# ParsaEsmati/SEA

Measured on AMD Instinct MI355X. Metric: rollout steps/sec (full-context forward, recompute mode) on cylinder_flow-shaped fields, higher is better.
Workload: dtype bf16

## Files before the change

sea_amd/csrc/mlp_block.hip:

```cpp
#include "gemm_core.hpp"
#include <stdlib.h>

struct MlpBlockLaunch {
    SeaMlpGroup g1[SEA_MAX_MLP_GROUPS];
    SeaMlp2Group g2[SEA_MAX_MLP_GROUPS];
    int tile_start[SEA_MAX_MLP_GROUPS + 1];
    int xcd_start[SEA_MAX_MLP_GROUPS + 1];
    int n_groups;
    float eps;
    int per_xcd;
    int probe;
};

__device__ __forceinline__ void glds16_blk(const void* gsrc, unsigned lds_addr) {
    unsigned keep;
    asm volatile("s_mov_b32 %0, m0\n\ts_mov_b32 m0, %2\n\ts_nop 0\n\tglobal_load_lds_dwordx4 %1, off\n\ts_mov_b32 m0, %0"
                 : "=&s"(keep) : "v"(gsrc), "s"(lds_addr) : "memory");
}

__device__ __forceinline__ void glds16_blk_s(const void* ubase, unsigned lane_off, unsigned lds_addr) {
    unsigned keep;
    asm volatile("s_mov_b32 %0, m0\n\ts_mov_b32 m0, %3\n\ts_nop 0\n\tglobal_load_lds_dwordx4 %1, %2\n\ts_mov_b32 m0, %0"
                 : "=&s"(keep) : "v"(lane_off), "s"(ubase), "s"(lds_addr) : "memory");
}

template <int KT, int NSB>
struct MlpBlockCfg {
    static constexpr int BM = 32, BKB = 128, NS = 4, NW = 8;
    static constexpr int E = KT * 64, S = NSB * 128;
    static constexpr int A_BYTES = KT * BM * BKB, STAGE = KT * 64 * BKB;
    static constexpr int PRM_OFF = A_BYTES + NS * STAGE;
    static constexpr int P1_BYTES = PRM_OFF + 2 * S * 4;
    static constexpr int SLAB_PITCH = 128 * 4 + 16, SLAB = BM * SLAB_PITCH;
    static constexpr int X3_OFF = NW * SLAB;
    static constexpr int RED2_OFF = X3_OFF + KT * BM * BKB;
    static constexpr int P2_BYTES = RED2_OFF + 2 * NW * BM * 4;
    static constexpr int RS = KT == 4 ? 8 : 4, SLOT = 16 * 128;
    static constexpr int RING_OFF = KT == 4 ? A_BYTES : P1_BYTES;
    static constexpr int RING_END = RING_OFF + NW * RS * SLOT;
    static constexpr int BYTES_ = P1_BYTES > P2_BYTES ? P1_BYTES : P2_BYTES;
    static constexpr int BYTES = BYTES_ > RING_END ? BYTES_ : RING_END;
};

__device__ __forceinline__ f32x4 mma16_first(const uint4& a, const uint4& b) {
    return __builtin_amdgcn_mfma_f32_16x16x32_bf16(__builtin_bit_cast(bf16x8, a), __builtin_bit_cast(bf16x8, b), f32x4{0.f, 0.f, 0.f, 0.f}, 0, 0, 0);
}

__device__ __forceinline__ constexpr int blk_col_base(int t, int half, int wq) { return (t >> 1) * 512 + half * 256 + wq * 64 + (t & 1) * 32; }

template <int KT, int NSB>
__global__ __launch_bounds__(512) void mlp_block_kernel(const MlpBlockLaunch L) {
    using T = __bf16;
    using Cf = MlpBlockCfg<KT, NSB>;
    constexpr int BM = 32, BKB = 128, BK = 64, NS = 4, NW = 8;
    constexpr int E = Cf::E, S = Cf::S, NSTAGE = S / 64, NT = NSB / 2;
    constexpr int A_BYTES = Cf::A_BYTES, STAGE = Cf::STAGE;
    constexpr int LPS = KT * 8 / NW;
    constexpr int PRM_OFF = Cf::PRM_OFF;
    constexpr int B1_OFF = 0, RED_OFF = S * 4;
    static_assert(RED_OFF + 2 * NW * BM * 4 <= A_BYTES && (S / 256) * 1024 <= A_BYTES && LPS * NW == KT * 8 && NT % 2 == 0 && Cf::BYTES <= 160 * 1024, "LDS layout of sea_mlp_block");
    static_assert((NT / 2) * 512 == S, "blk_col_base covers the hidden columns once");
    extern __shared__ __attribute__((aligned(16))) char smem[];
    int tile, gi = 0;
    if (L.per_xcd < 0) {
        const int xcd = (int)(blockIdx.x & 7), idx = (int)(blockIdx.x >> 3);
        if (xcd >= L.xcd_start[L.n_groups]) return;
        while (gi + 1 < L.n_groups && xcd >= L.xcd_start[gi + 1]) ++gi;
        tile = L.tile_start[gi] + (xcd - L.xcd_start[gi]) * 32 + idx;
        if (tile >= L.tile_start[gi + 1]) return;
    } else {
        tile = L.per_xcd > 0 ? (int)(blockIdx.x & 7) * L.per_xcd + (int)(blockIdx.x >> 3) : (int)blockIdx.x;
        if (tile >= L.tile_start[L.n_groups]) return;
        while (gi + 1 < L.n_groups && tile >= L.tile_start[gi + 1]) ++gi;
    }
    const SeaMlpGroup& G = L.g1[gi];
    const SeaMlp2Group& H = L.g2[gi];
    const int m0 = (tile - L.tile_start[gi]) * BM, M = G.M;
    const int tid = threadIdx.x, lane = tid & 63;
    const int wave = __builtin_amdgcn_readfirstlane(tid >> 6);
    const int r = lane & 15, g = lane >> 4;
    const int half = wave >> 2, wq = wave & 3;
    const T* A = static_cast<const T*>(G.A);
    const T* W = static_cast<const T*>(G.W1);
    const unsigned lds_base = __builtin_amdgcn_readfirstlane((unsigned)(uintptr_t)smem);
    const int rl = lane >> 3;
    const int chunk = (lane & 7) ^ (rl & 7);
    for (int p = wave; p < 2 * (S / 256); p += NW) {
        const float* src = p < S / 256 ? G.lnw : G.lnb;
        const int q = p < S / 256 ? p : p - S / 256;
        glds16_blk(src + q * 256 + lane * 4, lds_base + (unsigned)(PRM_OFF + p * 1024));
    }
    for (int p = wave; G.X32 == nullptr && p < KT * (BM / 8); p += NW) {
        const int kt = p / (BM / 8), u = p - kt * (BM / 8);
        int row = m0 + u * 8 + rl;
        row = row < M ? row : M - 1;
        glds16_blk(A + (int64_t)row * G.lda + kt * BK + chunk * 8, lds_base + (unsigned)(kt * BM * BKB + u * 8 * BKB));
    }
    const unsigned w1_lane = (unsigned)(((8 * (rl >> 2) + (rl & 3)) * G.ldw + chunk * 8) * 2);
    auto dma_stage = [&](int s) {
        const unsigned base = lds_base + (unsigned)(A_BYTES + (s % NS) * STAGE);
        const int t = s >> 2, u = (s >> 1) & 1, hs = s & 1;
#pragma unroll
        for (int i = 0; i < LPS; ++i) {
            const int p = i * NW + wave;
            const int kt = p >> 3, u8 = p & 7;
            const int urow = blk_col_base(t, hs, u8 >> 1) + 16 * (u8 & 1) + 4 * u;
            glds16_blk_s(W + (int64_t)urow * G.ldw + kt * BK, w1_lane, base + (unsigned)(kt * 64 * BKB + u8 * 8 * BKB));
        }
    };
    dma_stage(0);
    if (G.X32 != nullptr) {
        constexpr int CPT = E / 16;
        const int prow = tid >> 4, pl = tid & 15;
        int row = m0 + prow;
        row = row < M ? row : M - 1;
        const int c0 = pl * CPT;
        float xv[CPT];
#pragma unroll
        for (int c = 0; c < CPT; c += 4) load4(G.X32 + (int64_t)row * G.ldx32 + c0 + c, *reinterpret_cast<float(*)[4]>(xv + c));
        if (G.addend != nullptr) {
#pragma unroll
            for (int c = 0; c < CPT; c += 4) {
                float av[4];
                load4(G.addend + (int64_t)row * G.ldadd + c0 + c, av);
#pragma unroll
                for (int e = 0; e < 4; ++e) xv[c + e] += av[e];
            }
        }
        float gq[CPT], bq[CPT];
#pragma unroll
        for (int c = 0; c < CPT; c += 4) {
            load4(G.gamma + c0 + c, *reinterpret_cast<float(*)[4]>(gq + c));
#pragma unroll
            for (int e = 0; e < 4; ++e) bq[c + e] = 0.f;
            if (G.beta != nullptr) load4(G.beta + c0 + c, *reinterpret_cast<float(*)[4]>(bq + c));
            if (G.mod != nullptr) {
                float mw[4], mb[4];
                const T* mod = static_cast<const T*>(G.mod) + (int64_t)row * G.ldmod;
                load4(mod + c0 + c, mw);
                load4(mod + E + c0 + c, mb);
#pragma unroll
                for (int e = 0; e < 4; ++e) {
                    gq[c + e] += 1.0f + mw[e];
                    bq[c + e] += mb[e];
                }
            }
        }
        float s4[4] = {0.f, 0.f, 0.f, 0.f};
#pragma unroll
        for (int c = 0; c < CPT; c += 4)
#pragma unroll
            for (int e = 0; e < 4; ++e) s4[e] = add1(s4[e], xv[c + e]);
        float sm_ = add1(add1(s4[0], s4[1]), add1(s4[2], s4[3]));
#pragma unroll
        for (int o = 8; o >= 1; o >>= 1) sm_ += __shfl_xor(sm_, o);
        const float mean = sm_ * (1.0f / (float)E);
        float q4[4] = {0.f, 0.f, 0.f, 0.f};
#pragma unroll
        for (int c = 0; c < CPT; c += 4)
#pragma unroll
            for (int e = 0; e < 4; ++e) {
                const float d_ = xv[c + e] - mean;
                q4[e] = fma1(d_, d_, q4[e]);
            }
        float sq = add1(add1(q4[0], q4[1]), add1(q4[2], q4[3]));
#pragma unroll
        for (int o = 8; o >= 1; o >>= 1) sq += __shfl_xor(sq, o);
        const float rstd = 1.0f / sqrtf(sq * (1.0f / (float)E) + G.norm_eps);
#pragma unroll
        for (int c = 0; c < CPT; c += 8) {
            const int col = c0 + c, kt = col >> 6, ck = (col & 63) >> 3;
            bf16x8 pv;
#pragma unroll
            for (int e = 0; e < 8; ++e) pv[e] = (__bf16)((xv[c + e] - mean) * rstd * gq[c + e] + bq[c + e]);
            *reinterpret_cast<bf16x8*>(smem + kt * BM * BKB + prow * BKB + ((ck ^ (prow & 7)) << 4)) = pv;
        }
        asm volatile("s_waitcnt vmcnt(0) lgkmcnt(0)" ::: "memory");
    }
    for (int s = 1; s < NS - 1; ++s) dma_stage(s);

    const T* W2 = static_cast<const T*>(H.W2);
    const unsigned w2_lane = (unsigned)((rl * H.ldw2 + chunk * 8) * 2);
    const T* Wp = static_cast<const T*>(H.Wproj);
    const unsigned wp_lane = (unsigned)((rl * H.ldwp + chunk * 8) * 2);
    constexpr int NSLOT = (E / 16) * (NT / 2);
    constexpr int NJ = E / NW / 16;
    constexpr int NX = NJ * KT;
    auto w2_slot = [&](int k) {
        const unsigned dst = lds_base + (unsigned)(Cf::RING_OFF + (wave * Cf::RS + (k % Cf::RS)) * Cf::SLOT);
        if (k < NSLOT) {
            const int tau = k / (E / 16), j = k - tau * (E / 16);
            const T* ub = W2 + (int64_t)(j * 16) * H.ldw2 + blk_col_base(2 * tau, half, wq);
#pragma unroll
            for (int u = 0; u < 2; ++u)
                glds16_blk_s(ub + (int64_t)(8 * u) * H.ldw2, w2_lane, dst + (unsigned)(u * 1024));
        } else {
            const int kk = k - NSLOT, j = kk / KT, kt = kk - j * KT;
            const T* ub = Wp + (int64_t)(wave * (E / NW) + j * 16) * H.ldwp + kt * BK;
#pragma unroll
            for (int u = 0; u < 2; ++u)
                glds16_blk_s(ub + (int64_t)(8 * u) * H.ldwp, wp_lane, dst + (unsigned)(u * 1024));
        }
    };
    uint4 hid[NT][2];
    float mean[2], rstd[2];
    {
        f32x4 acc[NSB][2];
        uint4 areg[KT][2][2];
#pragma unroll
        for (int i = 0; i < NSB; ++i) {
            acc[i][0] = f32x4{0.f, 0.f, 0.f, 0.f};
            acc[i][1] = f32x4{0.f, 0.f, 0.f, 0.f};
        }
#pragma unroll
        for (int s = 0; s < NSTAGE; ++s) {
            if (s + 2 < NSTAGE) asm volatile("s_waitcnt vmcnt(%0) lgkmcnt(0)" ::"n"(2 * LPS) : "memory");
            else if (s + 1 < NSTAGE) asm volatile("s_waitcnt vmcnt(%0) lgkmcnt(0)" ::"n"(LPS) : "memory");
            else asm volatile("s_waitcnt vmcnt(0) lgkmcnt(0)" ::: "memory");
            __builtin_amdgcn_s_barrier();
            if (s + NS - 1 < NSTAGE) dma_stage(s + NS - 1);
            if (s == 0) {
                const char* sA = smem + r * BKB;
#pragma unroll
                for (int kt = 0; kt < KT; ++kt)
#pragma unroll
                    for (int kc = 0; kc < 2; ++kc) {
                        const int off = ((kc * 4 + g) ^ (r & 7)) << 4;
                        areg[kt][kc][0] = *reinterpret_cast<const uint4*>(sA + kt * BM * BKB + off);
                        areg[kt][kc][1] = *reinterpret_cast<const uint4*>(sA + kt * BM * BKB + 16 * BKB + off);
                    }
                asm volatile("s_waitcnt lgkmcnt(0)" ::: "memory");
            }
            if (s == 1)
                for (int p = wave; p < S / 256; p += NW) glds16_blk(G.b1 + p * 256 + lane * 4, lds_base + (unsigned)(B1_OFF + p * 1024));
            if ((s & 1) == half) {
                const char* sW = smem + A_BYTES + (s % NS) * STAGE + (wq * 16 + r) * BKB;
#pragma unroll
                for (int kt = 0; kt < KT; ++kt)
#pragma unroll
                    for (int kc = 0; kc < 2; ++kc) {
                        const int off = ((kc * 4 + g) ^ (r & 7)) << 4;
                        const uint4 wf = *reinterpret_cast<const uint4*>(sW + kt * 64 * BKB + off);
                        mma16<T>(wf, areg[kt][kc][0], acc[s >> 1][0]);
                        mma16<T>(wf, areg[kt][kc][1], acc[s >> 1][1]);
                    }
            }
        }
        if (L.probe == 1) return;
        float* red = reinterpret_cast<float*>(smem + RED_OFF);
        const float* pb1 = reinterpret_cast<const float*>(smem + B1_OFF);
        const float* pgm = reinterpret_cast<const float*>(smem + PRM_OFF);
        const float* pbt = pgm + S;
        const float inv_s = 1.0f / (float)S;
        float sum[2] = {0.f, 0.f};
#pragma unroll
        for (int i = 0; i < NSB; ++i) {
            const int n = blk_col_base(i >> 1, half, wq) + 8 * g + 4 * (i & 1);
            float bv[4];
            load4(pb1 + n, bv);
#pragma unroll
            for (int mb = 0; mb < 2; ++mb) {
#pragma unroll
                for (int q = 0; q < 4; ++q) acc[i][mb][q] += bv[q];
                sum[mb] += (acc[i][mb][0] + acc[i][mb][1]) + (acc[i][mb][2] + acc[i][mb][3]);
            }
        }
#pragma unroll
        for (int mb = 0; mb < 2; ++mb) {
            sum[mb] += __shfl_xor(sum[mb], 16);
            sum[mb] += __shfl_xor(sum[mb], 32);
            if (g == 0) red[wave * 32 + mb * 16 + r] = sum[mb];
        }
        __syncthreads();
#pragma unroll
        for (int k = 0; k < Cf::RS - 1; ++k) w2_slot(k);
        float sq[2] = {0.f, 0.f};
#pragma unroll
        for (int mb = 0; mb < 2; ++mb) {
            float t = 0.f;
#pragma unroll
            for (int w = 0; w < NW; ++w) t += red[w * 32 + mb * 16 + r];
            mean[mb] = t * inv_s;
        }
#pragma unroll
        for (int i = 0; i < NSB; ++i)
#pragma unroll
            for (int mb = 0; mb < 2; ++mb)
#pragma unroll
                for (int q = 0; q < 4; ++q) {
                    const float c = acc[i][mb][q] - mean[mb];
                    sq[mb] += c * c;
                }
#pragma unroll
        for (int mb = 0; mb < 2; ++mb) {
            sq[mb] += __shfl_xor(sq[mb], 16);
            sq[mb] += __shfl_xor(sq[mb], 32);
            if (g == 0) red[256 + wave * 32 + mb * 16 + r] = sq[mb];
        }
        asm volatile("s_waitcnt lgkmcnt(0)" ::: "memory");
        __builtin_amdgcn_s_barrier();
#pragma unroll
        for (int mb = 0; mb < 2; ++mb) {
            float t = 0.f;
#pragma unroll
            for (int w = 0; w < NW; ++w) t += red[256 + w * 32 + mb * 16 + r];
            rstd[mb] = 1.0f / sqrtf(t * inv_s + L.eps);
        }
#pragma unroll
        for (int i = 0; i < NSB; ++i) {
            const int n = blk_col_base(i >> 1, half, wq) + 8 * g + 4 * (i & 1);
            float gm[4], bt[4];
            load4(pgm + n, gm);
            load4(pbt + n, bt);
#pragma unroll
            for (int mb = 0; mb < 2; ++mb) {
                bf16x4 y;
#pragma unroll
                for (int q = 0; q < 4; ++q) y[q] = (__bf16)gelu_erf_bf16((acc[i][mb][q] - mean[mb]) * rstd[mb] * gm[q] + bt[q]);
                uint2 y2 = *reinterpret_cast<const uint2*>(&y);
                asm volatile("" : "+v"(y2.x), "+v"(y2.y));
                if (i & 1) {
                    hid[i >> 1][mb].z = y2.x;
                    hid[i >> 1][mb].w = y2.y;
                } else {
                    hid[i >> 1][mb].x = y2.x;
                    hid[i >> 1][mb].y = y2.y;
                }
            }
            __builtin_amdgcn_sched_barrier(0);
        }
    }
    __builtin_amdgcn_sched_barrier(0);
    if (L.probe == 2) {
        asm volatile("s_waitcnt vmcnt(0)" ::: "memory");
        return;
    }

    constexpr int NJB = E / 16;
    constexpr int NTOT = NSLOT + NX;
    f32x4 acc2[2][NJB];
    uint4 wp[KT * 2][NJ];
#pragma unroll
    for (int k = 0; k < NTOT; ++k) {
        const int tau = k / NJB, j = k - tau * NJB;
        {
            constexpr int AFTER_MAX = Cf::RS - 2;
            const int after = NTOT - 1 - k < AFTER_MAX ? NTOT - 1 - k : AFTER_MAX;
            switch (after) {
                case 6: asm volatile("s_waitcnt vmcnt(12) lgkmcnt(0)" ::: "memory"); break;
                case 5: asm volatile("s_waitcnt vmcnt(10) lgkmcnt(0)" ::: "memory"); break;
                case 4: asm volatile("s_waitcnt vmcnt(8) lgkmcnt(0)" ::: "memory"); break;
                case 3: asm volatile("s_waitcnt vmcnt(6) lgkmcnt(0)" ::: "memory"); break;
                case 2: asm volatile("s_waitcnt vmcnt(4) lgkmcnt(0)" ::: "memory"); break;
                case 1: asm volatile("s_waitcnt vmcnt(2) lgkmcnt(0)" ::: "memory"); break;
                default: asm volatile("s_waitcnt vmcnt(0) lgkmcnt(0)" ::: "memory"); break;
            }
        }
        if (k + Cf::RS - 1 < NTOT) w2_slot(k + Cf::RS - 1);
        const char* sl = smem + Cf::RING_OFF + (wave * Cf::RS + (k % Cf::RS)) * Cf::SLOT + r * 128;
        if (k >= NSLOT) {
            const int kk = k - NSLOT, jp = kk / KT, kt = kk - jp * KT;
#pragma unroll
            for (int kc = 0; kc < 2; ++kc) wp[kt * 2 + kc][jp] = *reinterpret_cast<const uint4*>(sl + (((kc * 4 + g) ^ (r & 7)) << 4));
            continue;
        }
#pragma unroll
        for (int u2 = 0; u2 < 2; ++u2) {
            const uint4 w = *reinterpret_cast<const uint4*>(sl + (((u2 * 4 + g) ^ (r & 7)) << 4));
            const int t = 2 * tau + u2;
            if (t == 0) {
                acc2[0][j] = mma16_first(w, hid[0][0]);
                acc2[1][j] = mma16_first(w, hid[0][1]);
            } else {
                mma16<T>(w, hid[t][0], acc2[0][j]);
                mma16<T>(w, hid[t][1], acc2[1][j]);
            }
        }
        __builtin_amdgcn_sched_barrier(0);
    }
    __syncthreads();
    if (L.probe == 3) return;
    {
    int tid_l = threadIdx.x;
    asm volatile("" : "+v"(tid_l));
    const int tid = tid_l, lane = tid & 63, r = lane & 15, g = lane >> 4;
    (void)lane;
    constexpr int NH = E / 128, JH = 8;
    const int srow = tid >> 4, scb = (tid & 15) * 8;
    float resv[NH][8];
    {
        int row = m0 + srow;
        row = row < M ? row : M - 1;
#pragma unroll
        for (int h = 0; h < NH; ++h) {
            const int col = h * 128 + scb;
            float b2a[4], b2b[4];
            load4(H.b2 + col, b2a);
            load4(H.b2 + col + 4, b2b);
            float ra[4], rb[4];
            if (H.R != nullptr) {
                load4(H.R + (int64_t)row * H.ldr + col, ra);
                load4(H.R + (int64_t)row * H.ldr + col + 4, rb);
            } else {
                load4(G.X32 + (int64_t)row * G.ldx32 + col, ra);
                load4(G.X32 + (int64_t)row * G.ldx32 + col + 4, rb);
                if (G.addend != nullptr) {
                    float aa[4], ab[4];
                    load4(G.addend + (int64_t)row * G.ldadd + col, aa);
                    load4(G.addend + (int64_t)row * G.ldadd + col + 4, ab);
#pragma unroll
                    for (int q = 0; q < 4; ++q) {
                        ra[q] += aa[q];
                        rb[q] += ab[q];
                    }
                }
            }
#pragma unroll
            for (int q = 0; q < 4; ++q) {
                resv[h][q] = b2a[q] + ra[q];
                resv[h][4 + q] = b2b[q] + rb[q];
            }
        }
    }
    constexpr int CPT = E / 16;
    const int ec0 = (tid & 15) * CPT;
    float ebp[CPT], egq[CPT], ebq[CPT];
    const bool has_norm = H.gamma != nullptr;
#pragma unroll
    for (int h = 0; h < NH; ++h) {
        char* slab = smem + wave * Cf::SLAB;
#pragma unroll
        for (int mb = 0; mb < 2; ++mb)
#pragma unroll
            for (int j = 0; j < JH; ++j)
                *reinterpret_cast<f32x4*>(slab + (mb * 16 + r) * Cf::SLAB_PITCH + (j * 16 + g * 4) * 4) = acc2[mb][h * JH + j];
        if (h == NH - 1) {
            __builtin_amdgcn_sched_barrier(0);
            int m = m0 + srow;
            m = m < M ? m : M - 1;
#pragma unroll
            for (int c = 0; c < CPT; c += 4) {
                load4(H.bproj + ec0 + c, *reinterpret_cast<float(*)[4]>(ebp + c));
#pragma unroll
                for (int q = 0; q < 4; ++q) egq[c + q] = ebq[c + q] = 0.f;
                if (has_norm) {
                    load4(H.gamma + ec0 + c, *reinterpret_cast<float(*)[4]>(egq + c));
                    if (H.beta != nullptr) load4(H.beta + ec0 + c, *reinterpret_cast<float(*)[4]>(ebq + c));
                    if (H.mod != nullptr) {
                        float mw[4], mb[4];
                        const T* mod = static_cast<const T*>(H.mod) + (int64_t)m * H.ldmod;
                        load4(mod + ec0 + c, mw);
                        load4(mod + E + ec0 + c, mb);
#pragma unroll
                        for (int q = 0; q < 4; ++q) {
                            egq[c + q] += 1.0f + mw[q];
                            ebq[c + q] += mb[q];
                        }
                    }
                }
            }
        }
        asm volatile("s_waitcnt lgkmcnt(0)" ::: "memory");
        __builtin_amdgcn_s_barrier();
        {
            float v[8];
#pragma unroll
            for (int q = 0; q < 8; ++q) v[q] = resv[h][q];
#pragma unroll
            for (int w = 0; w < NW; ++w) {
                const float4 a = *reinterpret_cast<const float4*>(smem + w * Cf::SLAB + srow * Cf::SLAB_PITCH + scb * 4);
                const float4 b = *reinterpret_cast<const float4*>(smem + w * Cf::SLAB + srow * Cf::SLAB_PITCH + scb * 4 + 16);
                v[0] += a.x; v[1] += a.y; v[2] += a.z; v[3] += a.w;
                v[4] += b.x; v[5] += b.y; v[6] += b.z; v[7] += b.w;
            }
            const int col = h * 128 + scb, kt = col >> 6, ck = (col & 63) >> 3;
            bf16x8 pv;
#pragma unroll
            for (int q = 0; q < 8; ++q) pv[q] = (__bf16)v[q];
            *reinterpret_cast<bf16x8*>(smem + Cf::X3_OFF + kt * BM * BKB + srow * BKB + ((ck ^ (srow & 7)) << 4)) = pv;
        }
        asm volatile("s_waitcnt lgkmcnt(0)" ::: "memory");
        __builtin_amdgcn_s_barrier();
        if (L.probe == 5 + h) return;
    }

    if (L.probe == 4) return;
    f32x4 acc3[2][NJ];
    {
        const char* sA = smem + Cf::X3_OFF + r * BKB;
#pragma unroll
        for (int kt = 0; kt < KT; ++kt)
#pragma unroll
            for (int kc = 0; kc < 2; ++kc) {
                const int off = ((kc * 4 + g) ^ (r & 7)) << 4;
                const uint4 af0 = *reinterpret_cast<const uint4*>(sA + kt * BM * BKB + off);
                const uint4 af1 = *reinterpret_cast<const uint4*>(sA + kt * BM * BKB + 16 * BKB + off);
#pragma unroll
                for (int j = 0; j < NJ; ++j) {
                    if (kt == 0 && kc == 0) {
                        acc3[0][j] = mma16_first(wp[0][j], af0);
                        acc3[1][j] = mma16_first(wp[0][j], af1);
                    } else {
                        mma16<T>(wp[kt * 2 + kc][j], af0, acc3[0][j]);
                        mma16<T>(wp[kt * 2 + kc][j], af1, acc3[1][j]);
                    }
                }
            }
    }
    constexpr int SEG = 80, YP = (E / 16) * SEG + 16;
    static_assert(BM * YP <= Cf::X3_OFF, "the y tile lies in front of the x3 tile");
#pragma unroll
    for (int i = 0; i < 2; ++i)
#pragma unroll
        for (int j = 0; j < NJ; ++j) {
            const int n = wave * (E / NW) + j * 16 + g * 4;
            *reinterpret_cast<f32x4*>(smem + (i * 16 + r) * YP + (n >> 4) * SEG + (n & 15) * 4) = acc3[i][j];
        }
    asm volatile("s_waitcnt lgkmcnt(0)" ::: "memory");
    __builtin_amdgcn_s_barrier();
    {
        float v[CPT];
#pragma unroll
        for (int c = 0; c < CPT; c += 4) {
            const float4 y = *reinterpret_cast<const float4*>(smem + srow * YP + ((ec0 + c) >> 4) * SEG + ((ec0 + c) & 15) * 4);
            v[c] = y.x + ebp[c]; v[c + 1] = y.y + ebp[c + 1]; v[c + 2] = y.z + ebp[c + 2]; v[c + 3] = y.w + ebp[c + 3];
        }
        if (has_norm) {
            float s4[4] = {0.f, 0.f, 0.f, 0.f};
#pragma unroll
            for (int c = 0; c < CPT; c += 4)
#pragma unroll
                for (int e = 0; e < 4; ++e) s4[e] = add1(s4[e], v[c + e]);
            float sm_ = add1(add1(s4[0], s4[1]), add1(s4[2], s4[3]));
#pragma unroll
            for (int o = 8; o >= 1; o >>= 1) sm_ += __shfl_xor(sm_, o);
            const float mean2 = sm_ * (1.0f / (float)E);
            float q4[4] = {0.f, 0.f, 0.f, 0.f};
#pragma unroll
            for (int c = 0; c < CPT; c += 4)
#pragma unroll
                for (int e = 0; e < 4; ++e) {
                    const float d_ = v[c + e] - mean2;
                    q4[e] = fma1(d_, d_, q4[e]);
                }
            float sq = add1(add1(q4[0], q4[1]), add1(q4[2], q4[3]));
#pragma unroll
            for (int o = 8; o >= 1; o >>= 1) sq += __shfl_xor(sq, o);
            const float rstd2 = 1.0f / sqrtf(sq * (1.0f / (float)E) + L.eps);
#pragma unroll
            for (int c = 0; c < CPT; ++c) v[c] = (v[c] - mean2) * rstd2 * egq[c] + ebq[c];
        }
        const int m = m0 + srow;
        if (m < M) {
#pragma unroll
            for (int c = 0; c < CPT; c += 4) {
                if (H.Y32 != nullptr) store4(H.Y32 + (int64_t)m * H.ldy32 + ec0 + c, v[c], v[c + 1], v[c + 2], v[c + 3]);
                if (H.Yact != nullptr) store4(static_cast<T*>(H.Yact) + (int64_t)m * H.ldyact + ec0 + c, v[c], v[c + 1], v[c + 2], v[c + 3]);
            }
        }
    }
    }
}

extern "C" int sea_mlp_block(const SeaMlpGroup* g1, const SeaMlp2Group* g2, int n_groups, float eps, int dtype, void* stream) {
    SEA_REQUIRE(g1 != nullptr && g2 != nullptr && n_groups >= 1 && n_groups <= SEA_MAX_MLP_GROUPS, "sea_mlp_block: n_groups=%d out of range", n_groups);
    const int E = g1[0].E, S = g1[0].S;
    const bool shape_ok = (E == 256 && S == 2048) || (E == 128 && S == 1024);
    if (dtype != SEA_BF16 || !shape_ok) {
        sea_set_error("sea_mlp_block: unsupported dtype / shape (dtype=%d E=%d S=%d): bf16, (E, S) in {(256, 2048), (128, 1024)}", dtype, E, S);
        return SEA_EUNSUPPORTED;
    }
    MlpBlockLaunch L;
    memset(&L, 0, sizeof(L));
    int total = 0;
    for (int i = 0; i < n_groups; ++i) {
        const SeaMlpGroup& G = g1[i];
        const SeaMlp2Group& H = g2[i];
        SEA_REQUIRE(G.E == E && G.S == S && H.E == E && H.S == S && G.M >= 1 && H.M == G.M, "sea_mlp_block[%d]: the groups of a launch share E and S; both halves the same M", i);
        SEA_REQUIRE((G.A || G.X32) && G.W1 && G.b1 && G.lnw && G.lnb, "sea_mlp_block[%d]: null pointer (first layer)", i);
        SEA_REQUIRE((G.X32 || (G.lda % 8 == 0 && G.lda >= E)) && G.ldw % 8 == 0 && G.ldw >= E, "sea_mlp_block[%d]: bad strides (first layer)", i);
        if (G.X32 != nullptr)
            SEA_REQUIRE(G.gamma && G.ldx32 % 4 == 0 && G.ldx32 >= E && (!G.addend || (G.ldadd % 4 == 0 && G.ldadd >= E)) && G.Xout == nullptr &&
                            (!G.mod || (G.ldmod % 8 == 0 && G.ldmod >= 2 * E)) && sea_aligned16(G.X32) && sea_aligned16(G.addend) && sea_aligned16(G.mod) &&
                            sea_aligned16(G.gamma) && sea_aligned16(G.beta) && G.norm_eps > 0.f,
                        "sea_mlp_block[%d]: norm prologue: null / misaligned pointer, bad stride, or Xout (the block keeps x + addend to itself)", i);
        SEA_REQUIRE(sea_aligned16(G.A) && sea_aligned16(G.W1) && sea_aligned16(G.b1) && sea_aligned16(G.lnw) && sea_aligned16(G.lnb), "sea_mlp_block[%d]: pointers must be 16-byte aligned", i);
        SEA_REQUIRE(H.W2 && H.b2 && (H.R || G.X32) && H.Wproj && H.bproj && (H.Y32 || H.Yact), "sea_mlp_block[%d]: null pointer (second layer; R may be NULL with the norm prologue: the residual is then x + addend)", i);
        SEA_REQUIRE(H.ldw2 % 8 == 0 && H.ldw2 >= S && H.ldwp % 8 == 0 && H.ldwp >= E && (!H.R || (H.ldr % 4 == 0 && H.ldr >= E)) &&
                        (!H.Y32 || (H.ldy32 % 4 == 0 && H.ldy32 >= E)) && (!H.Yact || (H.ldyact % 4 == 0 && H.ldyact >= E)) && (!H.mod || (H.ldmod % 4 == 0 && H.ldmod >= 2 * E)),
                    "sea_mlp_block[%d]: bad strides (second layer)", i);
        SEA_REQUIRE(sea_aligned16(H.W2) && sea_aligned16(H.b2) && sea_aligned16(H.R) && sea_aligned16(H.Wproj) && sea_aligned16(H.bproj) && sea_aligned16(H.gamma) && sea_aligned16(H.beta) &&
                        sea_aligned16(H.mod) && sea_aligned16(H.Y32) && sea_aligned16(H.Yact),
                    "sea_mlp_block[%d]: pointers must be 16-byte aligned", i);
        SEA_REQUIRE(H.gamma || (!H.beta && !H.mod), "sea_mlp_block[%d]: beta / mod without gamma", i);
        L.g1[i] = G;
        L.g2[i] = H;
        L.tile_start[i] = total;
        total += (G.M + 31) / 32;
    }
    L.tile_start[n_groups] = total;
    L.n_groups = n_groups;
    L.eps = eps;
    static const int probe = sea_tune("blk_probe", 0);
    L.probe = probe;
    hipStream_t s = static_cast<hipStream_t>(stream);
    int xcds = 0;
    for (int i = 0; i < n_groups; ++i) {
        L.xcd_start[i] = xcds;
        xcds += (L.tile_start[i + 1] - L.tile_start[i] + 31) / 32;
    }
    L.xcd_start[n_groups] = xcds;
    static const int xcd_excl = sea_tune("blk_xcd", 0);
    static const int per_xcd_on = sea_tune("blk_perxcd", 1);
    if (total > 256 && per_xcd_on) {
        L.per_xcd = (total + 7) / 8;
        total = 8 * L.per_xcd;
    } else if (xcds <= 8 && xcd_excl) {
        L.per_xcd = -1;
        total = 256;
    }
    if (E == 256) {
        constexpr int lds = MlpBlockCfg<4, 16>::BYTES;
        static const hipError_t once = hipFuncSetAttribute(reinterpret_cast<const void*>(mlp_block_kernel<4, 16>), hipFuncAttributeMaxDynamicSharedMemorySize, lds);
        (void)once;
        mlp_block_kernel<4, 16><<<dim3(total), dim3(512), lds, s>>>(L);
    } else {
        constexpr int lds = MlpBlockCfg<2, 8>::BYTES;
        static const hipError_t once = hipFuncSetAttribute(reinterpret_cast<const void*>(mlp_block_kernel<2, 8>), hipFuncAttributeMaxDynamicSharedMemorySize, lds);
        (void)once;
        mlp_block_kernel<2, 8><<<dim3(total), dim3(512), lds, s>>>(L);
    }
    SEA_CHECK_LAUNCH("sea_mlp_block");
    sea_note_form("mlp_block.rows32", L.per_xcd, total);
    return SEA_OK;
}
```

Before: 5643.

## Stream W1 through per-wave LDS ring instead of shared block-wide stages

Replaces the block-wide four-stage W1 staging, which needed a barrier every stage, with a per-wave ring of eight slots. Each wave now loads only its own W1 tiles and waits on vmcnt without block barriers. The W2 ring continues in the same slots, and W2 prefetch now starts before the LayerNorm reduction. This cuts synchronisation in the first GEMM and overlaps W2 loads with the normalisation, at the cost of a fixed ring size for every KT, a changed LDS layout and extra code for a probe mode.

```diff
diff --git a/sea_amd/csrc/mlp_block.hip b/sea_amd/csrc/mlp_block.hip
--- a/sea_amd/csrc/mlp_block.hip
+++ b/sea_amd/csrc/mlp_block.hip
@@ -26,21 +26,31 @@
 
 template <int KT, int NSB>
 struct MlpBlockCfg {
-    static constexpr int BM = 32, BKB = 128, NS = 4, NW = 8;
+    static constexpr int BM = 32, BKB = 128, NW = 8;
     static constexpr int E = KT * 64, S = NSB * 128;
-    static constexpr int A_BYTES = KT * BM * BKB, STAGE = KT * 64 * BKB;
-    static constexpr int PRM_OFF = A_BYTES + NS * STAGE;
+    static constexpr int A_BYTES = KT * BM * BKB;
+    static constexpr int RS = 8, SLOT = 16 * 128;
+    static constexpr int RING_OFF = A_BYTES;
+    static constexpr int PRM_OFF = RING_OFF + NW * RS * SLOT;
     static constexpr int P1_BYTES = PRM_OFF + 2 * S * 4;
     static constexpr int SLAB_PITCH = 128 * 4 + 16, SLAB = BM * SLAB_PITCH;
     static constexpr int X3_OFF = NW * SLAB;
     static constexpr int RED2_OFF = X3_OFF + KT * BM * BKB;
     static constexpr int P2_BYTES = RED2_OFF + 2 * NW * BM * 4;
-    static constexpr int RS = KT == 4 ? 8 : 4, SLOT = 16 * 128;
-    static constexpr int RING_OFF = KT == 4 ? A_BYTES : P1_BYTES;
-    static constexpr int RING_END = RING_OFF + NW * RS * SLOT;
-    static constexpr int BYTES_ = P1_BYTES > P2_BYTES ? P1_BYTES : P2_BYTES;
-    static constexpr int BYTES = BYTES_ > RING_END ? BYTES_ : RING_END;
+    static constexpr int BYTES = P1_BYTES > P2_BYTES ? P1_BYTES : P2_BYTES;
 };
+
+__device__ __forceinline__ void ring_wait(int after) {
+    switch (after) {
+        case 6: asm volatile("s_waitcnt vmcnt(12) lgkmcnt(0)" ::: "memory"); break;
+        case 5: asm volatile("s_waitcnt vmcnt(10) lgkmcnt(0)" ::: "memory"); break;
+        case 4: asm volatile("s_waitcnt vmcnt(8) lgkmcnt(0)" ::: "memory"); break;
+        case 3: asm volatile("s_waitcnt vmcnt(6) lgkmcnt(0)" ::: "memory"); break;
+        case 2: asm volatile("s_waitcnt vmcnt(4) lgkmcnt(0)" ::: "memory"); break;
+        case 1: asm volatile("s_waitcnt vmcnt(2) lgkmcnt(0)" ::: "memory"); break;
+        default: asm volatile("s_waitcnt vmcnt(0) lgkmcnt(0)" ::: "memory"); break;
+    }
+}
 
 __device__ __forceinline__ f32x4 mma16_first(const uint4& a, const uint4& b) {
     return __builtin_amdgcn_mfma_f32_16x16x32_bf16(__builtin_bit_cast(bf16x8, a), __builtin_bit_cast(bf16x8, b), f32x4{0.f, 0.f, 0.f, 0.f}, 0, 0, 0);
@@ -52,14 +62,15 @@
 __global__ __launch_bounds__(512) void mlp_block_kernel(const MlpBlockLaunch L) {
     using T = __bf16;
     using Cf = MlpBlockCfg<KT, NSB>;
-    constexpr int BM = 32, BKB = 128, BK = 64, NS = 4, NW = 8;
-    constexpr int E = Cf::E, S = Cf::S, NSTAGE = S / 64, NT = NSB / 2;
-    constexpr int A_BYTES = Cf::A_BYTES, STAGE = Cf::STAGE;
-    constexpr int LPS = KT * 8 / NW;
+    constexpr int BM = 32, BKB = 128, BK = 64, NW = 8;
+    constexpr int E = Cf::E, S = Cf::S, NT = NSB / 2;
+    constexpr int A_BYTES = Cf::A_BYTES;
     constexpr int PRM_OFF = Cf::PRM_OFF;
     constexpr int B1_OFF = 0, RED_OFF = S * 4;
-    static_assert(RED_OFF + 2 * NW * BM * 4 <= A_BYTES && (S / 256) * 1024 <= A_BYTES && LPS * NW == KT * 8 && NT % 2 == 0 && Cf::BYTES <= 160 * 1024, "LDS layout of sea_mlp_block");
+    constexpr int N1 = NSB * KT;
+    static_assert(RED_OFF + 2 * NW * BM * 4 <= A_BYTES && (S / 256) * 1024 <= A_BYTES && NT % 2 == 0 && Cf::BYTES <= 160 * 1024, "LDS layout of sea_mlp_block");
     static_assert((NT / 2) * 512 == S, "blk_col_base covers the hidden columns once");
+    static_assert(N1 % Cf::RS == 0 && N1 >= Cf::RS && Cf::RS - 2 <= 6, "the W2 slots continue the ring at position 0; ring_wait counts up to six slots");
     extern __shared__ __attribute__((aligned(16))) char smem[];
     int tile, gi = 0;
     if (L.per_xcd < 0) {
@@ -97,18 +108,17 @@
         glds16_blk(A + (int64_t)row * G.lda + kt * BK + chunk * 8, lds_base + (unsigned)(kt * BM * BKB + u * 8 * BKB));
     }
     const unsigned w1_lane = (unsigned)(((8 * (rl >> 2) + (rl & 3)) * G.ldw + chunk * 8) * 2);
-    auto dma_stage = [&](int s) {
-        const unsigned base = lds_base + (unsigned)(A_BYTES + (s % NS) * STAGE);
-        const int t = s >> 2, u = (s >> 1) & 1, hs = s & 1;
-#pragma unroll
-        for (int i = 0; i < LPS; ++i) {
-            const int p = i * NW + wave;
-            const int kt = p >> 3, u8 = p & 7;
-            const int urow = blk_col_base(t, hs, u8 >> 1) + 16 * (u8 & 1) + 4 * u;
-            glds16_blk_s(W + (int64_t)urow * G.ldw + kt * BK, w1_lane, base + (unsigned)(kt * 64 * BKB + u8 * 8 * BKB));
-        }
+    auto w1_slot = [&](int n) {
+        const int i = n / KT, kt = n - i * KT;
+        const unsigned dst = lds_base + (unsigned)(Cf::RING_OFF + (wave * Cf::RS + (n % Cf::RS)) * Cf::SLOT);
+        const T* ub = W + (int64_t)(blk_col_base(i >> 1, half, wq) + 4 * (i & 1)) * G.ldw + kt * BK;
+#pragma unroll
+        for (int p = 0; p < 2; ++p)
+            glds16_blk_s(ub + (int64_t)(16 * p) * G.ldw, w1_lane, dst + (unsigned)(p * 1024));
     };
-    dma_stage(0);
+    constexpr int PRE = 2;
+#pragma unroll
+    for (int n = 0; n < PRE; ++n) w1_slot(n);
     if (G.X32 != nullptr) {
         constexpr int CPT = E / 16;
         const int prow = tid >> 4, pl = tid & 15;
@@ -177,7 +187,8 @@
         }
         asm volatile("s_waitcnt vmcnt(0) lgkmcnt(0)" ::: "memory");
     }
-    for (int s = 1; s < NS - 1; ++s) dma_stage(s);
+#pragma unroll
+    for (int n = PRE; n < Cf::RS - 1; ++n) w1_slot(n);
 
     const T* W2 = static_cast<const T*>(H.W2);
     const unsigned w2_lane = (unsigned)((rl * H.ldw2 + chunk * 8) * 2);
@@ -207,46 +218,50 @@
     {
         f32x4 acc[NSB][2];
         uint4 areg[KT][2][2];
-#pragma unroll
-        for (int i = 0; i < NSB; ++i) {
-            acc[i][0] = f32x4{0.f, 0.f, 0.f, 0.f};
-            acc[i][1] = f32x4{0.f, 0.f, 0.f, 0.f};
-        }
-#pragma unroll
-        for (int s = 0; s < NSTAGE; ++s) {
-            if (s + 2 < NSTAGE) asm volatile("s_waitcnt vmcnt(%0) lgkmcnt(0)" ::"n"(2 * LPS) : "memory");
-            else if (s + 1 < NSTAGE) asm volatile("s_waitcnt vmcnt(%0) lgkmcnt(0)" ::"n"(LPS) : "memory");
-            else asm volatile("s_waitcnt vmcnt(0) lgkmcnt(0)" ::: "memory");
-            __builtin_amdgcn_s_barrier();
-            if (s + NS - 1 < NSTAGE) dma_stage(s + NS - 1);
-            if (s == 0) {
-                const char* sA = smem + r * BKB;
-#pragma unroll
-                for (int kt = 0; kt < KT; ++kt)
-#pragma unroll
-                    for (int kc = 0; kc < 2; ++kc) {
-                        const int off = ((kc * 4 + g) ^ (r & 7)) << 4;
-                        areg[kt][kc][0] = *reinterpret_cast<const uint4*>(sA + kt * BM * BKB + off);
-                        areg[kt][kc][1] = *reinterpret_cast<const uint4*>(sA + kt * BM * BKB + 16 * BKB + off);
-                    }
-                asm volatile("s_waitcnt lgkmcnt(0)" ::: "memory");
-            }
-            if (s == 1)
-                for (int p = wave; p < S / 256; p += NW) glds16_blk(G.b1 + p * 256 + lane * 4, lds_base + (unsigned)(B1_OFF + p * 1024));
-            if ((s & 1) == half) {
-                const char* sW = smem + A_BYTES + (s % NS) * STAGE + (wq * 16 + r) * BKB;
-#pragma unroll
-                for (int kt = 0; kt < KT; ++kt)
-#pragma unroll
-                    for (int kc = 0; kc < 2; ++kc) {
-                        const int off = ((kc * 4 + g) ^ (r & 7)) << 4;
-                        const uint4 wf = *reinterpret_cast<const uint4*>(sW + kt * 64 * BKB + off);
-                        mma16<T>(wf, areg[kt][kc][0], acc[s >> 1][0]);
-                        mma16<T>(wf, areg[kt][kc][1], acc[s >> 1][1]);
-                    }
-            }
+        asm volatile("s_waitcnt vmcnt(%0) lgkmcnt(0)" ::"n"(2 * (Cf::RS - 1)) : "memory");
+        __builtin_amdgcn_s_barrier();
+        {
+            const char* sA = smem + r * BKB;
+#pragma unroll
+            for (int kt = 0; kt < KT; ++kt)
+#pragma unroll
+                for (int kc = 0; kc < 2; ++kc) {
+                    const int off = ((kc * 4 + g) ^ (r & 7)) << 4;
+                    areg[kt][kc][0] = *reinterpret_cast<const uint4*>(sA + kt * BM * BKB + off);
+                    areg[kt][kc][1] = *reinterpret_cast<const uint4*>(sA + kt * BM * BKB + 16 * BKB + off);
+                }
+        }
+        asm volatile("s_waitcnt lgkmcnt(0)" ::: "memory");
+        __builtin_amdgcn_s_barrier();
+        for (int p = wave; p < S / 256; p += NW) glds16_blk(G.b1 + p * 256 + lane * 4, lds_base + (unsigned)(B1_OFF + p * 1024));
+        if (L.probe == 7) {
+            asm volatile("s_waitcnt vmcnt(0)" ::: "memory");
+            return;
+        }
+#pragma unroll
+        for (int n = 0; n < N1; ++n) {
+            const int i = n / KT, kt = n - i * KT;
+            ring_wait(N1 - 1 - n < Cf::RS - 2 ? N1 - 1 - n : Cf::RS - 2);
+            if (n + Cf::RS - 1 < N1) w1_slot(n + Cf::RS - 1);
+            const char* sl = smem + Cf::RING_OFF + (wave * Cf::RS + (n % Cf::RS)) * Cf::SLOT + r * 128;
+#pragma unroll
+            for (int kc = 0; kc < 2; ++kc) {
+                const uint4 wf = *reinterpret_cast<const uint4*>(sl + (((kc * 4 + g) ^ (r & 7)) << 4));
+                if (kt == 0 && kc == 0) {
+                    acc[i][0] = mma16_first(wf, areg[0][0][0]);
+                    acc[i][1] = mma16_first(wf, areg[0][0][1]);
+                } else {
+                    mma16<T>(wf, areg[kt][kc][0], acc[i][0]);
+                    mma16<T>(wf, areg[kt][kc][1], acc[i][1]);
+                }
+            }
+            __builtin_amdgcn_sched_barrier(0);
         }
         if (L.probe == 1) return;
+        asm volatile("s_waitcnt lgkmcnt(0)" ::: "memory");
+#pragma unroll
+        for (int k = 0; k < Cf::RS - 1; ++k) w2_slot(k);
+        __builtin_amdgcn_s_barrier();
         float* red = reinterpret_cast<float*>(smem + RED_OFF);
         const float* pb1 = reinterpret_cast<const float*>(smem + B1_OFF);
         const float* pgm = reinterpret_cast<const float*>(smem + PRM_OFF);
@@ -271,9 +286,8 @@
             sum[mb] += __shfl_xor(sum[mb], 32);
             if (g == 0) red[wave * 32 + mb * 16 + r] = sum[mb];
         }
-        __syncthreads();
-#pragma unroll
-        for (int k = 0; k < Cf::RS - 1; ++k) w2_slot(k);
+        asm volatile("s_waitcnt lgkmcnt(0)" ::: "memory");
+        __builtin_amdgcn_s_barrier();
         float sq[2] = {0.f, 0.f};
 #pragma unroll
         for (int mb = 0; mb < 2; ++mb) {
@@ -343,19 +357,7 @@
 #pragma unroll
     for (int k = 0; k < NTOT; ++k) {
         const int tau = k / NJB, j = k - tau * NJB;
-        {
-            constexpr int AFTER_MAX = Cf::RS - 2;
-            const int after = NTOT - 1 - k < AFTER_MAX ? NTOT - 1 - k : AFTER_MAX;
-            switch (after) {
-                case 6: asm volatile("s_waitcnt vmcnt(12) lgkmcnt(0)" ::: "memory"); break;
-                case 5: asm volatile("s_waitcnt vmcnt(10) lgkmcnt(0)" ::: "memory"); break;
-                case 4: asm volatile("s_waitcnt vmcnt(8) lgkmcnt(0)" ::: "memory"); break;
-                case 3: asm volatile("s_waitcnt vmcnt(6) lgkmcnt(0)" ::: "memory"); break;
-                case 2: asm volatile("s_waitcnt vmcnt(4) lgkmcnt(0)" ::: "memory"); break;
-                case 1: asm volatile("s_waitcnt vmcnt(2) lgkmcnt(0)" ::: "memory"); break;
-                default: asm volatile("s_waitcnt vmcnt(0) lgkmcnt(0)" ::: "memory"); break;
-            }
-        }
+        ring_wait(NTOT - 1 - k < Cf::RS - 2 ? NTOT - 1 - k : Cf::RS - 2);
         if (k + Cf::RS - 1 < NTOT) w2_slot(k + Cf::RS - 1);
         const char* sl = smem + Cf::RING_OFF + (wave * Cf::RS + (k % Cf::RS)) * Cf::SLOT + r * 128;
         if (k >= NSLOT) {
```

Result: faster. 5713, median of 5 (+1.2%).
